# prime-slam/octreelib

Measured on AMD Instinct MI355X. Metric: Mpoints/s insert+subdivide+RANSAC, higher is better.
Workload: dtype f64; 1 GPU; BASELINE config 3: Grid 1 m voxels, 10000000 planar points per GPU (scene 32x32x32 voxels), insert + subdivide(len>64) + map_leaf_points_cuda_ransac(H=1024, k=6, thr=0.01, poses_per_batch=10) incl. apply_mask; points_per_gpu=10000000, K=64, hypotheses=1024, leaves=575543

## Files before the change

### octreelib_amd/csrc/common.h

```cpp
#pragma once

#include <hip/hip_runtime.h>
#include <stdint.h>

#include <cstdio>
#include <cstring>
#include <map>
#include <string>
#include <vector>

#include "../../include/octreelib_hip.h"

#include <atomic>
extern std::atomic<uint64_t> g_octl_host_syncs;
static inline hipError_t octl_counted_stream_sync(hipStream_t s) {
  g_octl_host_syncs.fetch_add(1, std::memory_order_relaxed);
  return hipStreamSynchronize(s);
}
static inline hipError_t octl_counted_event_sync(hipEvent_t e) {
  g_octl_host_syncs.fetch_add(1, std::memory_order_relaxed);
  return hipEventSynchronize(e);
}
#define hipStreamSynchronize(s) octl_counted_stream_sync(s)
#define hipEventSynchronize(e) octl_counted_event_sync(e)
// ... 81 lines not shown
  hipEvent_t self_gate = nullptr, self_done = nullptr;
  struct Upload { const char* dst; size_t bytes; hipEvent_t done; };
  std::vector<Upload> uploads;
  std::vector<DevBuf> pool;
  size_t pool_bytes = 0;
  std::map<void*, size_t> user_blocks;
  unsigned char geom_hint[192] = {0};
  bool geom_hint_valid = false;
  bool geom_hint_staged = false;
  struct octl_forest* pending_mask_forest = nullptr;
  uint64_t geom_hint_want = 0;
  bool geom_hint_two_pass = false;
  bool geom_sparse = false;
  bool had_chunks = false;
  int64_t spec_points = 0, spec_nodes = 0, spec_vox = 0, spec_blocks = 0;
  DevBuf hyp_dev;
  DevBuf f32_stage;
  DevBuf ls_buf;
  DevBuf rs_counters;
  int rs_parity = 0;
  uint32_t wait_seq = 0;
  bool rs_counters_dirty = false;
  std::vector<double> hyp_host;
  void* comm = nullptr;
  int n_ranks = 1, rank = 0;
  DevBuf routed_xyz, routed_gidx;
  bool routed_taken = false;
  DevBuf rt_hist, rt_counts, rt_matrix, rt_send_xyz, rt_send_gidx;
  int64_t routed_n = 0;
};

int octl_set_error(octl_ctx* ctx, int code, const char* fmt, ...);
enum { MIRROR_COPY_WORDS = 512, MIRROR_BBOX_WORD = 896, MIRROR_RS_VIOLATION = 990, MIRROR_MASK_TOTALS = 992,
       MIRROR_FLAG_BUILD = 1000, MIRROR_FLAG_MASK0 = 1001, MIRROR_FLAG_MASK1 = 1002 };
static_assert(MIRROR_COPY_WORDS <= MIRROR_BBOX_WORD && MIRROR_BBOX_WORD + 8 <= MIRROR_RS_VIOLATION &&
              MIRROR_RS_VIOLATION < MIRROR_MASK_TOTALS &&
              MIRROR_MASK_TOTALS + 2 <= MIRROR_FLAG_BUILD && MIRROR_FLAG_MASK1 < 1024, "mirror layout");
enum {
  SM_ERR = 0,
  SM_BBOX = 4,
  SM_NVOX = 12,
  SM_NSPLIT = 13,
  SM_NTILES = 14,
  SM_ETOTAL = 15,
  SM_NBLOCKS = 16,
  SM_BK_TICKET = 17,
// ... 95 lines not shown
```

### octreelib_amd/csrc/ctx.hip

```cpp
#include <chrono>
#include <cstdarg>
#include <cstdlib>

#include <algorithm>

#include "common.h"

int octl_set_error(octl_ctx* ctx, int code, const char* fmt, ...) {
  char buf[1024];
  va_list ap;
  va_start(ap, fmt);
  vsnprintf(buf, sizeof(buf), fmt, ap);
  va_end(ap);
  if (ctx) ctx->err = buf;
  return code;
}

std::atomic<uint64_t> g_octl_host_syncs{0};

namespace {
struct OptName { const char* name; int64_t OctlOptions::*field; };
const OptName kOptions[] = {
    {"NO_BUCKET_BUILD", &OctlOptions::no_bucket_build},     {"BUCKET_POINTS", &OctlOptions::bucket_points},
    {"SYNC_GEOM", &OctlOptions::sync_geom},                 {"NO_GEOM_HINT", &OctlOptions::no_geom_hint},
// ... 342 lines not shown
}

int octl_comm_destroy(octl_ctx* ctx);

void octl_ctx_destroy(octl_ctx* ctx) {
  if (!ctx) return;
  (void)hipSetDevice(ctx->device);
  (void)hipStreamSynchronize(ctx->stream);
  if (ctx->comm) (void)octl_comm_destroy(ctx);
  for (auto& pe : ctx->pending) {
    (void)hipEventDestroy(pe.start);
    (void)hipEventDestroy(pe.stop);
  }
  for (auto ev : ctx->event_pool) (void)hipEventDestroy(ev);
  if (ctx->handoff_event) (void)hipEventDestroy(ctx->handoff_event);
  for (auto ev : ctx->pin_event)
    if (ev) (void)hipEventDestroy(ev);
  for (auto& pb : ctx->pool) (void)hipFree(pb.p);
  ctx->pool.clear();
  for (auto& ub : ctx->user_blocks) (void)hipFree(ub.first);
  ctx->user_blocks.clear();
  for (auto& b : ctx->scan_tmp) devbuf_free(b);
  devbuf_free(ctx->hyp_dev);
  devbuf_free(ctx->f32_stage);
  devbuf_free(ctx->ls_buf);
  devbuf_free(ctx->rs_counters);
  devbuf_free(ctx->scan_status);
  devbuf_free(ctx->small);
  devbuf_free(ctx->routed_xyz);
  devbuf_free(ctx->routed_gidx);
  for (DevBuf* b : {&ctx->rt_hist, &ctx->rt_counts, &ctx->rt_matrix, &ctx->rt_send_xyz,
                    &ctx->rt_send_gidx})
    devbuf_free(*b);
  if (ctx->small_host) (void)hipHostFree(ctx->small_host);
  if (ctx->pinned) (void)hipHostFree(ctx->pinned);
  if (ctx->self_stream) {
    (void)hipStreamSynchronize(ctx->self_stream);
    (void)hipStreamDestroy(ctx->self_stream);
    if (ctx->self_gate) (void)hipEventDestroy(ctx->self_gate);
    if (ctx->self_done) (void)hipEventDestroy(ctx->self_done);
  }
  if (ctx->copy_stream) {
    (void)hipStreamSynchronize(ctx->copy_stream);
    (void)hipStreamDestroy(ctx->copy_stream);
  }
  if (ctx->copy_gate) (void)hipEventDestroy(ctx->copy_gate);
// ... 163 lines not shown
```

### octreelib_amd/csrc/forest.h

```cpp
#pragma once
#include "common.h"

#define OCTL_VOX_BIAS (1 << 20)
#define OCTL_VOX_ABS_LIMIT (1 << 30)
#define OCTL_VOX_DEAD (~0ull)
struct VoxOrg {
  int32_t x = 0, y = 0, z = 0;
};
__host__ __device__ static inline uint64_t vkey_pack(int64_t qx, int64_t qy, int64_t qz, const VoxOrg& g) {
  return ((uint64_t)(qx - g.x + OCTL_VOX_BIAS) << 42) | ((uint64_t)(qy - g.y + OCTL_VOX_BIAS) << 21) |
         (uint64_t)(qz - g.z + OCTL_VOX_BIAS);
}
__host__ __device__ static inline bool vkey_in_window(int64_t qx, int64_t qy, int64_t qz, const VoxOrg& g) {
  const int64_t ax = qx - g.x, ay = qy - g.y, az = qz - g.z;
  return ax > -OCTL_VOX_BIAS && ax < OCTL_VOX_BIAS && ay > -OCTL_VOX_BIAS && ay < OCTL_VOX_BIAS &&
         az > -OCTL_VOX_BIAS && az < OCTL_VOX_BIAS;
}
__host__ __device__ static inline void vkey_decode(uint64_t k, const VoxOrg& g, int64_t q[3]) {
  q[0] = (int64_t)((k >> 42) & 0x1FFFFF) - OCTL_VOX_BIAS + g.x;
  q[1] = (int64_t)((k >> 21) & 0x1FFFFF) - OCTL_VOX_BIAS + g.y;
  q[2] = (int64_t)(k & 0x1FFFFF) - OCTL_VOX_BIAS + g.z;
}

struct NodeTable {
// ... 82 lines not shown
  DevBuf bk_table;
  DevBuf bk_tot;
  DevBuf bk_chunks;
  DevBuf bk_vox;
  DevBuf bk_node;
  DevBuf leafinfo;
  struct LevelSeg { int64_t a, b; int depth; };
  std::vector<LevelSeg> level_segs;
  DevBuf vkey, path, lin[2], val[2], hist, idxbuf[2], pathbuf[2], flags, entries, split[2],
      split_tiles[2], child_sc, pose_off_dev, scheme_dev, root_up;
};

int forest_build(octl_forest* f, int64_t K, const uint8_t* scheme_mask, int32_t n_mask,
                 int32_t keep_scheme, int32_t max_depth, octl_build_info* info, const PlanarRule* planar = nullptr);
int planar_level_stats(octl_forest* f, const PlanarRule& rule, NodeTable& nt, int64_t first_new, int64_t n_new,
                       const uint32_t* idx, const double* xyz, int xs, int64_t n_alive);
int nodes_reserve(octl_ctx* ctx, NodeTable& t, int64_t cap);
void nodes_free(octl_ctx* ctx, NodeTable& t);

int ransac_launch(octl_ctx* ctx, const double* xyz_dev, int64_t n_points,
                  const uint32_t* blk_start, const int32_t* blk_size, const int32_t* order_dev,
                  int64_t nb, const double* hyp_dev, int32_t H, int32_t k, double thr,
                  uint8_t* mask_dev, float* plane_dev, int32_t* count_dev, int32_t* index_dev,
                  uint8_t* evaluated_dev, DevBuf& scratch, int64_t max_block = INT64_MAX);
int ransac_check_table(octl_ctx* ctx, const double* hyp, int32_t H, int32_t k);
int store_adopt(octl_forest* f, DevBuf& src, int64_t n, bool* adopted);
int store_compute_bbox(octl_forest* f);
int store_materialize(octl_forest* f);
int bbox_ensure(octl_forest* f);
int alive_ensure(octl_forest* f);
int forest_make_blocks(octl_forest* f);
int forest_finish_blocks(octl_forest* f, uint32_t* err_out);
int forest_sync_vkeys(octl_forest* f);
int forest_fix_origin(octl_forest* f, const int bb[6]);
int forest_sync_vcodes(octl_forest* f);
int forest_insert_incremental(octl_forest* f, int* done, octl_build_info* info);

int forest_settle(octl_forest* f);
void forest_forget_pending(octl_forest* f);
int ensure_mask(octl_forest* f);
```

### octreelib_amd/csrc/mask.hip

```cpp
#include "forest.h"
#include "lookback.h"

namespace {

__device__ __forceinline__ void mask_tile_count(const uint8_t* __restrict__ mask, int64_t n,
                                                uint32_t* __restrict__ tilecnt, uint32_t tile,
                                                uint8_t* __restrict__ alive_fill) {
  __shared__ uint32_t s_w[4];
  const int64_t i0 = (int64_t)tile * 2048 + (int64_t)threadIdx.x * 8;
  uint32_t c = 0;
  if (i0 + 8 <= n) {
    const uint64_t w = *reinterpret_cast<const uint64_t*>(mask + i0);
    const uint64_t nz = ((w & 0x7F7F7F7F7F7F7F7Full) + 0x7F7F7F7F7F7F7F7Full) | w;
    c = (uint32_t)__popcll(nz & 0x8080808080808080ull);
    if (alive_fill) *reinterpret_cast<uint64_t*>(alive_fill + i0) = 0x0101010101010101ull;
  } else {
    for (int64_t i = i0; i < n; ++i) {
      c += mask[i] ? 1u : 0u;
      if (alive_fill) alive_fill[i] = 1;
    }
  }
#pragma unroll
  for (int off = 32; off > 0; off >>= 1) c += __shfl_xor(c, off);
  if ((threadIdx.x & 63) == 0) s_w[threadIdx.x >> 6] = c;
// ... 94 lines not shown
    if ((keepbits >> r) & 1u) {
      const int64_t d = (int64_t)toff + s_cnt[r * 4 + wave] + rk[r];
      ord_idx2[d] = iv[r];
      xyz_ord2[3 * d] = px[r];
      xyz_ord2[3 * d + 1] = py[r];
      xyz_ord2[3 * d + 2] = pz[r];
      if (alive_fill) alive_fill[iv[r]] = 1;
    } else {
      alive[iv[r]] = 0;
    }
  }
}

__global__ __launch_bounds__(256) void k_compact_tiles(
    const uint8_t* __restrict__ mask, const uint32_t* __restrict__ tile_off, int64_t n,
    const uint32_t* __restrict__ ord_idx, const double* __restrict__ xyz_ord,
    uint32_t* __restrict__ ord_idx2, double* __restrict__ xyz_ord2, uint8_t* __restrict__ alive) {
  __shared__ uint32_t s_cnt[33];
  compact_tile(blockIdx.x, mask, n, ord_idx, xyz_ord, ord_idx2, xyz_ord2, alive, nullptr, s_cnt,
               [&](uint32_t) { return tile_off[blockIdx.x]; });
}


__global__ __launch_bounds__(256) void k_mask_scan(
    const uint8_t* __restrict__ mask, int64_t n, uint32_t nt,
    const uint32_t* __restrict__ ord_idx, const double* __restrict__ xyz_ord,
    uint32_t* __restrict__ ord_idx2, double* __restrict__ xyz_ord2, uint8_t* __restrict__ alive,
    const uint32_t* __restrict__ blk_start, const int32_t* __restrict__ blk_size, int64_t nb,
    const int32_t* __restrict__ blk_node, const int32_t* __restrict__ blk_slot, int32_t* __restrict__ blk_node2,
    int32_t* __restrict__ blk_slot2, uint32_t* __restrict__ blk_start2, int32_t* __restrict__ blk_size2,
    uint64_t* __restrict__ st_tiles, uint64_t* __restrict__ st_kept, uint64_t* __restrict__ st_ids, uint32_t epoch,
    uint32_t* __restrict__ mirror, uint32_t seq, uint8_t* __restrict__ alive_fill) {
  __shared__ uint32_t s_w[2][4];
  __shared__ uint32_t s_excl;
  __shared__ uint32_t s_cnt[33];
  const int lane = threadIdx.x & 63, wave = threadIdx.x >> 6;
  if (blockIdx.x < nt) {
    const uint32_t tile = blockIdx.x;
    compact_tile(tile, mask, n, ord_idx, xyz_ord, ord_idx2, xyz_ord2, alive, alive_fill, s_cnt,
                 [&](uint32_t total) {
                   const uint32_t excl = lookback_exclusive(st_tiles, epoch, tile, total, &s_excl);
                   if (threadIdx.x == 0 && tile == nt - 1) {
                     mirror[MIRROR_MASK_TOTALS] = excl + total;
                     mirror_publish(mirror, MIRROR_FLAG_MASK0, seq);
                   }
                   return excl;
                 });
    return;
  }
  const uint32_t bw = blockIdx.x - nt;
  const int64_t b = (int64_t)bw * 256 + threadIdx.x;
  const uint32_t st = b < nb ? blk_start[b] : 0u;
  const int sz = b < nb ? blk_size[b] : 0;
  uint32_t c = 0;
  if (sz <= 256)
    for (int i = 0; i < sz; ++i) c += mask[(size_t)st + i] ? 1u : 0u;
  unsigned long long big = __ballot(sz > 256);
  while (big) {
    const int src = __ffsll((long long)big) - 1;
    big &= big - 1;
    const uint32_t s0 = (uint32_t)__shfl((int)st, src);
    const int z = __shfl(sz, src);
    uint32_t cc = 0;
    for (int i = lane; i < z; i += 64) cc += mask[(size_t)s0 + i] ? 1u : 0u;
#pragma unroll
    for (int off = 32; off > 0; off >>= 1) cc += __shfl_xor(cc, off);
    if (lane == src) c = cc;
  }
  const uint32_t ne = c ? 1u : 0u;
  uint32_t ic = c, ie = ne;
#pragma unroll
  for (int off = 1; off < 64; off <<= 1) {
    const uint32_t tc = __shfl_up(ic, off), te = __shfl_up(ie, off);
    if (lane >= off) {
      ic += tc;
      ie += te;
    }
  }
  if (lane == 63) {
    s_w[0][wave] = ic;
    s_w[1][wave] = ie;
  }
  __syncthreads();
  uint32_t pc = ic - c, pe = ie - ne, tot_c = 0, tot_e = 0;
#pragma unroll
  for (int w = 0; w < 4; ++w) {
    if (w < wave) {
      pc += s_w[0][w];
      pe += s_w[1][w];
    }
    tot_c += s_w[0][w];
    tot_e += s_w[1][w];
  }
  __syncthreads();
  const uint32_t ex_c = lookback_exclusive(st_kept, epoch, bw, tot_c, &s_excl);
  __syncthreads();
  const uint32_t ex_e = lookback_exclusive(st_ids, epoch, bw, tot_e, &s_excl);
  if (threadIdx.x == 0 && bw == gridDim.x - nt - 1) {
    mirror[MIRROR_MASK_TOTALS + 1] = ex_e + tot_e;
    mirror_publish(mirror, MIRROR_FLAG_MASK1, seq);
  }
  if (b < nb && c) {
    const uint32_t id = ex_e + pe;
    blk_node2[id] = blk_node[b];
    blk_slot2[id] = blk_slot[b];
    blk_start2[id] = ex_c + pc;
    blk_size2[id] = (int32_t)c;
  }
}

__global__ __launch_bounds__(256) void k_blk_compact(
    const uint32_t* __restrict__ raw, const uint32_t* __restrict__ scanned, const uint32_t* __restrict__ grand_total,
    int64_t nt, int64_t nb, const int32_t* __restrict__ blk_node,
    const int32_t* __restrict__ blk_slot, int32_t* __restrict__ blk_node2, int32_t* __restrict__ blk_slot2,
    uint32_t* __restrict__ blk_start2, int32_t* __restrict__ blk_size2, uint32_t* __restrict__ mirror,
    uint32_t seq) {
  const int64_t b = (int64_t)blockIdx.x * blockDim.x + threadIdx.x;
  const uint32_t base_kept = scanned[nt], base_id = scanned[nt + nb];
  if (b == 0) {
    mirror[MIRROR_MASK_TOTALS] = base_id - base_kept;
    mirror[MIRROR_MASK_TOTALS + 1] = *grand_total - base_id;
    mirror_publish(mirror, MIRROR_FLAG_MASK0, seq);
    mirror_publish(mirror, MIRROR_FLAG_MASK1, seq);
  }
  if (b >= nb) return;
  const uint32_t c = raw[nt + b];
  if (!c) return;
  const uint32_t id = scanned[nt + nb + b] - base_id;
  blk_node2[id] = blk_node[b];
  blk_slot2[id] = blk_slot[b];
// ... 14 lines not shown
  for (int64_t i = threadIdx.x & 63; i < n; i += 64) mask[s0 + i] = 0;
}

int apply_device_mask(octl_forest* f, int64_t* n_alive_out, bool async = false) {
  octl_ctx* ctx = f->ctx;
  hipStream_t st = ctx->stream;
  if (ctx->pending_mask_forest && ctx->pending_mask_forest != f) OCTL_TRY(forest_settle(ctx->pending_mask_forest));
  OCTL_TRY(forest_settle(f));
  const int64_t n = f->n_ord, nb = f->n_blocks;
  f->mask_valid = false;
  f->fast_order_valid = false;
  f->pooled_valid = false;
  if (n > 0 && nb > 0) {
    KTimer t(ctx, "apply_mask");
    uint32_t* small = ctx->small.as<uint32_t>();
    const int64_t nt = ceil_div(n, 2048);
    const int64_t n_all = nt + 2 * nb;
    const size_t o_out = (((size_t)n_all + 8) * 4 + 15) & ~(size_t)15;
    OCTL_TRY(devbuf_reserve(ctx, f->flags, 2 * o_out));
    uint32_t* raw = f->flags.as<uint32_t>();
    uint32_t* scanned = reinterpret_cast<uint32_t*>(static_cast<char*>(f->flags.p) + o_out);
    const uint8_t* mask = f->mask.as<uint8_t>();
    const bool fused = !ctx->opt.no_fused_tables && nt + 2 * ceil_div(nb, 256) <= 1024;
    const uint32_t wait_seq = octl_wait_next_seq(ctx);
    uint8_t* fill = nullptr;
    if (f->alive_stale && f->n_ord == f->n_store) {
      fill = f->alive.as<uint8_t>();
      f->alive_stale = false;
    } else {
      OCTL_TRY(alive_ensure(f));
    }
    if (!fused) {
      OCTL_LAUNCH(k_blk_kept, dim3((unsigned)nt + grid_for(nb)), dim3(256), 0, st, mask, n, (uint32_t)nt, raw,
                         (const uint32_t*)f->blk_start.as<uint32_t>(), (const int32_t*)f->blk_size.as<int32_t>(), nb,
                         raw + nt, raw + nt + nb, fill);
      HIP_TRY(ctx, hipGetLastError());
      OCTL_TRY(octl_exclusive_scan_u32(ctx, raw, scanned, n_all, small + SM_MASK_TOTAL));
    }
    OCTL_TRY(devbuf_reserve(ctx, f->ord_idx2, (size_t)n * 4));
    OCTL_TRY(devbuf_reserve(ctx, f->xyz_ord2, (size_t)n * 24));
    OCTL_TRY(devbuf_reserve(ctx, f->blk_node2, (size_t)n * 4));
    OCTL_TRY(devbuf_reserve(ctx, f->blk_slot2, (size_t)n * 4));
    OCTL_TRY(devbuf_reserve(ctx, f->blk_start2, (size_t)n * 4));
    OCTL_TRY(devbuf_reserve(ctx, f->blk_size2, (size_t)n * 4));
    if (fused) {
      const int64_t nbw = ceil_div(nb, 256);
      uint64_t* status = nullptr;
      uint32_t epoch = 0;
      OCTL_TRY(octl_scan_status_acquire(ctx, nt + 2 * nbw, &status, &epoch));
      OCTL_LAUNCH(k_mask_scan, dim3((unsigned)(nt + nbw)), dim3(256), 0, st, mask, n, (uint32_t)nt,
                         (const uint32_t*)f->ord_idx.as<uint32_t>(), (const double*)f->xyz_ord.as<double>(),
                         f->ord_idx2.as<uint32_t>(), f->xyz_ord2.as<double>(), f->alive.as<uint8_t>(),
                         (const uint32_t*)f->blk_start.as<uint32_t>(), (const int32_t*)f->blk_size.as<int32_t>(), nb,
                         (const int32_t*)f->blk_node.as<int32_t>(), (const int32_t*)f->blk_slot.as<int32_t>(),
                         f->blk_node2.as<int32_t>(), f->blk_slot2.as<int32_t>(), f->blk_start2.as<uint32_t>(),
                         f->blk_size2.as<int32_t>(), status, status + nt, status + nt + nbw, epoch,
                         static_cast<uint32_t*>(ctx->small_host), wait_seq, fill);
      HIP_TRY(ctx, hipGetLastError());
    }
    if (!fused) {
      OCTL_LAUNCH(k_compact_tiles, dim3((unsigned)nt), dim3(256), 0, st, mask, (const uint32_t*)scanned, n,
                         (const uint32_t*)f->ord_idx.as<uint32_t>(), (const double*)f->xyz_ord.as<double>(),
                         f->ord_idx2.as<uint32_t>(), f->xyz_ord2.as<double>(), f->alive.as<uint8_t>());
      HIP_TRY(ctx, hipGetLastError());
      OCTL_LAUNCH(k_blk_compact, dim3(grid_for(nb)), dim3(256), 0, st, (const uint32_t*)raw,
                         (const uint32_t*)scanned, (const uint32_t*)(small + SM_MASK_TOTAL), nt, nb,
                         (const int32_t*)f->blk_node.as<int32_t>(), (const int32_t*)f->blk_slot.as<int32_t>(),
                         f->blk_node2.as<int32_t>(), f->blk_slot2.as<int32_t>(), f->blk_start2.as<uint32_t>(),
                         f->blk_size2.as<int32_t>(), static_cast<uint32_t*>(ctx->small_host), wait_seq);
      HIP_TRY(ctx, hipGetLastError());
    }
    std::swap(f->ord_idx, f->ord_idx2);
    std::swap(f->xyz_ord, f->xyz_ord2);
    std::swap(f->blk_node, f->blk_node2);
    std::swap(f->blk_slot, f->blk_slot2);
    std::swap(f->blk_start, f->blk_start2);
    std::swap(f->blk_size, f->blk_size2);
    f->totals_pending = true;
    f->totals_seq = wait_seq;
    f->totals_n_before = n;
    ctx->pending_mask_forest = f;
    if (!async) OCTL_TRY(forest_settle(f));
  }
  if (n_alive_out) *n_alive_out = f->n_ord;
  return OCTL_OK;
}

// ... 117 lines not shown
```

### octreelib_amd/csrc/order.hip

```cpp
#include <algorithm>

#include "forest.h"

namespace {

__global__ __launch_bounds__(256) void k_sub_up(const int32_t* __restrict__ first_child,
                                                int64_t a, int64_t b,
                                                uint32_t* __restrict__ nint) {
  const int64_t x = a + (int64_t)blockIdx.x * blockDim.x + threadIdx.x;
  if (x >= b) return;
  const int32_t fc = first_child[x];
  uint32_t s = 0;
  if (fc >= 0) {
    s = 1;
#pragma unroll
    for (int j = 0; j < 8; ++j) s += nint[fc + j];
  }
  nint[x] = s;
}

__global__ __launch_bounds__(256) void k_rank_down(const int32_t* __restrict__ first_child,
                                                   int64_t a, int64_t b,
                                                   const uint32_t* __restrict__ nint,
                                                   uint32_t* __restrict__ rank) {
// ... 283 lines not shown

extern "C" int octl_forest_ransac_all(octl_forest* f, int32_t poses_per_batch, const int32_t* e0,
                                      int32_t n_e0, const double* hypotheses, int32_t H, int32_t k,
                                      double threshold) {
  if (!f || !hypotheses) return OCTL_E_INVALID;
  OCTL_TRY(forest_settle(f));
  bool mask_fresh = false;
  const int rc = ransac_all_impl(f, poses_per_batch, e0, n_e0, hypotheses, H, k, threshold, &mask_fresh);
  if (mask_fresh) f->mask_valid = (rc == OCTL_OK);
  return rc;
}

static int ransac_all_impl(octl_forest* f, int32_t poses_per_batch, const int32_t* e0, int32_t n_e0,
                           const double* hypotheses, int32_t H, int32_t k, double threshold,
                           bool* mask_fresh) {
  octl_ctx* ctx = f->ctx;
  if (!f->built) return octl_set_error(ctx, OCTL_E_STATE, "ransac before build");
  if (poses_per_batch < 1) return octl_set_error(ctx, OCTL_E_INVALID, "poses_per_batch < 1");
  if (H < 1 || H > 1024 || k < 1) return octl_set_error(ctx, OCTL_E_INVALID, "bad H or k");
  OCTL_TRY(ransac_check_table(ctx, hypotheses, H, k));
  const int n_poses = (int)f->pose_off.size() - 1;
  if (e0 && n_e0 != n_poses) return octl_set_error(ctx, OCTL_E_INVALID, "e0 size mismatch");
  HIP_TRY(ctx, hipSetDevice(ctx->device));
  hipStream_t st = ctx->stream;
  if (!f->mask_valid) {
    OCTL_TRY(devbuf_reserve(ctx, f->mask, (size_t)std::max<int64_t>(f->n_ord, 1)));
    *mask_fresh = true;
  }
  if (f->n_blocks == 0) return OCTL_OK;
  const size_t hyp_cap_before = ctx->hyp_dev.cap;
  OCTL_TRY(devbuf_reserve(ctx, ctx->hyp_dev, (size_t)H * k * 8));
  const bool same_table = hyp_cap_before == ctx->hyp_dev.cap && ctx->hyp_host.size() == (size_t)H * k &&
                          std::memcmp(ctx->hyp_host.data(), hypotheses, (size_t)H * k * 8) == 0;
  if (same_table) {
  } else if ((size_t)H * k * 8 <= 64 * 1024) {
    char* pin = static_cast<char*>(ctx->pinned) + 128 * 1024;
    OCTL_TRY(pin_region_wait(ctx, 1));
    std::memcpy(pin, hypotheses, (size_t)H * k * 8);
    OCTL_TRY(octl_copy_from_pinned(ctx, ctx->hyp_dev.p, pin, (size_t)H * k * 8));
    OCTL_TRY(pin_region_mark(ctx, 1));
  } else {
    HIP_TRY(ctx, hipMemcpyAsync(ctx->hyp_dev.p, hypotheses, (size_t)H * k * 8, hipMemcpyHostToDevice, st));
    HIP_TRY(ctx, hipStreamSynchronize(st));
  }
  if (!same_table) ctx->hyp_host.assign(hypotheses, hypotheses + (size_t)H * k);
  const bool one_batch = n_poses <= poses_per_batch;
  std::vector<uint32_t> slot_counts;
  OCTL_TRY(forest_reference_order(f, e0, slot_counts, !one_batch));
  if (one_batch) {
    OCTL_TRY(ransac_launch(ctx, f->xyz_ord.as<double>(), f->n_ord, f->blk_start.as<uint32_t>(),
                           f->blk_size.as<int32_t>(), f->rs_order.as<int32_t>(), f->n_blocks,
                           ctx->hyp_dev.as<double>(), H, k, threshold, f->mask.as<uint8_t>(), nullptr,
                           nullptr, nullptr, nullptr, f->rs_scratch, f->max_block_hint));
    return OCTL_OK;
  }
  int64_t off = 0;
  for (int p0 = 0; p0 < n_poses; p0 += poses_per_batch) {
    int64_t nbatch = 0;
    for (int p = p0; p < std::min(n_poses, p0 + poses_per_batch); ++p) nbatch += slot_counts[p];
    if (nbatch > 0)
      OCTL_TRY(ransac_launch(ctx, f->xyz_ord.as<double>(), f->n_ord, f->blk_start.as<uint32_t>(),
                             f->blk_size.as<int32_t>(), f->rs_order.as<int32_t>() + off, nbatch,
                             ctx->hyp_dev.as<double>(), H, k, threshold, f->mask.as<uint8_t>(),
                             nullptr, nullptr, nullptr, nullptr, f->rs_scratch, f->max_block_hint));
    off += nbatch;
  }
  return OCTL_OK;
}
```

### octreelib_amd/csrc/ransac.hip

```cpp
#include <algorithm>
#include <cstdlib>
#include <type_traits>

#include "forest.h"
#include "lookback.h"
#include "wave_utils.h"

namespace {

__device__ __forceinline__ double div_by_small_int(double c, int k) {
  const double kd = (double)k;
  const double zh = 1.0 / kd;
  const double zl = fma(-kd, zh, 1.0) / kd;
  const double a = fabs(c);
  if (!((int(a > 1e-290) | int(c == 0.0)) & int(a < 1e290))) return c / kd;
  return copysign(fma(c, zh, c * zl), c);
}

__device__ __forceinline__ bool coord_in_fast_range(double v) {
  const uint32_t hi = (uint32_t)__double2hiint(v), lo = (uint32_t)__double2loint(v);
  const uint32_t e = (hi >> 20) & 0x7FFu;
  return (e - (1023u - 30u)) <= 60u || (hi | lo) == 0u;
}

// ... 1317 lines not shown
  if (bins[threadIdx.x]) atomicAdd(&counters[RC_BINS + threadIdx.x], bins[threadIdx.x]);
}

__device__ __forceinline__ void pos_table_entry(const double* __restrict__ hyp, int H, int k,
                                                uint2* __restrict__ tab, int n, int t) {
  const double* __restrict__ row = hyp + (int64_t)t * k;
  uint32_t x = 0, y = 0;
  for (int i = 0; i < k; ++i) {
    bool risky;
    const uint32_t g = (uint32_t)sample_index_cached(row[i], n, &risky);
    if (i < 4) x |= g << (8 * i); else y |= g << (8 * (i - 4));
    y |= (risky || g == (uint32_t)n) ? (0x10000u << i) : 0u;
  }
  tab[(size_t)n * (size_t)H + t] = uint2{x, y};
}
__device__ __forceinline__ void pos_table_part(const double* __restrict__ hyp, int H, int k,
                                               const uint32_t* __restrict__ counters, uint2* __restrict__ tab,
                                               int n, int part) {
  const int t = part * 256 + (int)threadIdx.x;
  if (t >= H || n < k || counters[RC_BINS + n] == 0u) return;
  pos_table_entry(hyp, H, k, tab, n, t);
}

__global__ __launch_bounds__(256) void k_block_scatter(const BlockDesc* __restrict__ desc, int64_t nb,
                                                       int cap, int k,
                                                       uint32_t* __restrict__ counters,
                                                       BlockDesc* __restrict__ sdesc, unsigned n_scatter,
                                                       const double* __restrict__ hyp, int H,
                                                       uint2* __restrict__ tab, uint32_t* __restrict__ next_counters) {
  if (next_counters && blockIdx.x == gridDim.x - 1)
    for (int w = threadIdx.x; w < RC_WORDS; w += blockDim.x) next_counters[w] = 0;
  if (blockIdx.x >= n_scatter) {
    const unsigned parts = (unsigned)(H + 255) / 256u;
    const unsigned id = blockIdx.x - n_scatter;
    pos_table_part(hyp, H, k, counters, tab, (int)(id / parts), (int)(id % parts));
    return;
  }
  __shared__ uint32_t cnt[256];
  __shared__ uint32_t base[256];
  __shared__ uint32_t c[256];
  cnt[threadIdx.x] = 0;
  c[threadIdx.x] = counters[RC_BINS + threadIdx.x];
  __syncthreads();
  uint32_t first = 0;
  for (int m = 255; m > (int)threadIdx.x; --m) first += c[m];
  if (blockIdx.x == 0) {
// ... 139 lines not shown
    first[m] = f;
    counters[RC_BINS + m] = cm;
    counters[RC_START + m] = f;
    if (m == 0) counters[RC_SORTED] = f + cm;
  }
  __syncthreads();
#pragma unroll
  for (int r = 0; r < BPS_PER_THREAD; ++r)
    if (dd[r].n >= 0) sdesc[first[dd[r].n] + rank[r]] = dd[r];
}

}

int ransac_check_table(octl_ctx* ctx, const double* hyp, int32_t H, int32_t k) {
  const int64_t n = (int64_t)H * k;
  for (int64_t i = 0; i < n; ++i)
    if (!(hyp[i] >= 0.0 && hyp[i] < 1.0))
      return octl_set_error(ctx, OCTL_E_INVALID,
                            "hypothesis table entry %lld = %g is outside [0, 1): the table must hold "
                            "np.random.random draws (cuda_ransac.py:39-41)", (long long)i, hyp[i]);
  return OCTL_OK;
}

int ransac_launch(octl_ctx* ctx, const double* xyz_dev, int64_t n_points,
                  const uint32_t* blk_start, const int32_t* blk_size, const int32_t* order_dev,
                  int64_t nb, const double* hyp_dev, int32_t H, int32_t k, double thr,
                  uint8_t* mask_dev, float* plane_dev, int32_t* count_dev, int32_t* index_dev,
                  uint8_t* evaluated_dev, DevBuf& scratch, int64_t max_block) {
  (void)evaluated_dev;
  if (nb <= 0) return OCTL_OK;
  if (H < 1 || H > 1024) return octl_set_error(ctx, OCTL_E_INVALID, "H must be in [1, 1024]");
  if (k < 1) return octl_set_error(ctx, OCTL_E_INVALID, "initial_points_number must be positive");
  const bool any_k = k > RS_KMAX;
  if (nb >= ((int64_t)1 << 31)) return octl_set_error(ctx, OCTL_E_INVALID, "too many blocks");
  hipStream_t st = ctx->stream;
  const size_t off_d = (((size_t)nb + 8) * 4 + 31) & ~(size_t)31;
  const size_t off_s = off_d + (size_t)nb * sizeof(BlockDesc);
  const size_t off_b = off_s + (size_t)nb * sizeof(BlockDesc);
  const size_t off_c = (off_b + (size_t)nb * 4 + 31) & ~(size_t)31;
  const bool use_tab = !any_k && k >= 3 && k <= 6 && (H > 256 || k == 6);
  const size_t off_t = (off_c + RC_WORDS * 4 + 31) & ~(size_t)31;
  OCTL_TRY(devbuf_reserve(ctx, scratch, off_t + (use_tab ? (size_t)256 * (size_t)H * sizeof(uint2) : 0)));
  char* base = static_cast<char*>(scratch.p);
  uint32_t* tmp = scratch.as<uint32_t>();
  BlockDesc* desc = reinterpret_cast<BlockDesc*>(base + off_d);
  BlockDesc* sdesc = reinterpret_cast<BlockDesc*>(base + off_s);
  uint32_t* big_list = reinterpret_cast<uint32_t*>(base + off_b);
  uint32_t* counters = reinterpret_cast<uint32_t*>(base + off_c);
  const bool fused = !ctx->opt.no_fused_tables;
  uint32_t* next_counters = nullptr;
  if (fused) {
    if (!ctx->rs_counters.p || ctx->rs_counters_dirty) {
      OCTL_TRY(devbuf_reserve(ctx, ctx->rs_counters, (size_t)2 * RC_WORDS * 4));
      HIP_TRY(ctx, hipMemsetAsync(ctx->rs_counters.p, 0, (size_t)2 * RC_WORDS * 4, st));
      ctx->rs_parity = 0;
    }
    counters = ctx->rs_counters.as<uint32_t>() + (size_t)ctx->rs_parity * RC_WORDS;
    next_counters = ctx->rs_counters.as<uint32_t>() + (size_t)(ctx->rs_parity ^ 1) * RC_WORDS;
    ctx->rs_parity ^= 1;
    ctx->rs_counters_dirty = true;
  }
  uint2* pos_tab = use_tab ? reinterpret_cast<uint2*>(base + off_t) : nullptr;
  const int threads = (H <= 64) ? 64 : (H <= 256 ? 256 : RS_BIG_THREADS);
  RansacOut out{mask_dev, plane_dev, count_dev, index_dev};
  if (fused && nb <= BPS_MAX) {
    KTimer t(ctx, "ransac_prepare");
    const int cap = any_k ? 0 : threads - 1;
    const unsigned n_table = use_tab && cap >= k ? (unsigned)(cap - k + 1) * (unsigned)ceil_div(H, BPS_THREADS) : 0u;
    auto kp = nb <= 2 * BPS_THREADS ? k_block_prepare_small<2>
              : (nb <= 4 * BPS_THREADS ? k_block_prepare_small<4>
                                       : (nb <= 6 * BPS_THREADS ? k_block_prepare_small<6> : k_block_prepare_small<8>));
    OCTL_LAUNCH(kp, dim3(1 + n_table), dim3(BPS_THREADS), 0, st, order_dev, blk_start, blk_size, nb,
                       n_points, cap, (int)k, desc, sdesc, big_list, counters, out, max_block,
                       static_cast<uint32_t*>(ctx->small_host), hyp_dev, (int)H, pos_tab, next_counters);
    HIP_TRY(ctx, hipGetLastError());
    ctx->rs_counters_dirty = false;
  } else {
    KTimer t(ctx, "ransac_prepare");
    if (fused) {
      const unsigned g = (unsigned)ceil_div(nb, 256 * BP_PER_THREAD);
      uint64_t* status = nullptr;
      uint32_t epoch = 0;
      OCTL_TRY(octl_scan_status_acquire(ctx, g, &status, &epoch));
      OCTL_LAUNCH(k_block_prepare, dim3(g), dim3(256), 0, st, order_dev, blk_start, blk_size, nb, n_points,
                         any_k ? 0 : threads - 1, (int)k, desc, big_list, counters, out, status, epoch, max_block,
                         static_cast<uint32_t*>(ctx->small_host));
      HIP_TRY(ctx, hipGetLastError());
    } else {
      const unsigned g = (unsigned)ceil_div(nb, 256);
      OCTL_LAUNCH(k_block_sizes_in_order, dim3(g), dim3(256), 0, st, order_dev, blk_size, nb, tmp, counters);
      HIP_TRY(ctx, hipGetLastError());
      OCTL_TRY(octl_exclusive_scan_u32(ctx, tmp, tmp, nb, nullptr));
      OCTL_LAUNCH(k_block_desc, dim3((unsigned)ceil_div(nb, 256 * BD_PER_THREAD)), dim3(256), 0, st, order_dev,
                         blk_start, blk_size,
                         (const uint32_t*)tmp, nb, n_points, any_k ? 0 : threads - 1, (int)k, desc, big_list,
                         counters, out);
      HIP_TRY(ctx, hipGetLastError());
    }
    const unsigned n_scatter = (unsigned)ceil_div(nb, 256 * BS_PER_THREAD);
    const unsigned n_table = use_tab ? 256u * (unsigned)ceil_div(H, 256) : 0u;
    OCTL_LAUNCH(k_block_scatter, dim3(n_scatter + n_table), dim3(256), 0, st,
                       (const BlockDesc*)desc, nb, any_k ? 0 : threads - 1, (int)k, counters, sdesc, n_scatter, hyp_dev,
                       (int)H, pos_tab, next_counters);
    HIP_TRY(ctx, hipGetLastError());
    ctx->rs_counters_dirty = false;
  }
  const int cus = octl_ctx_cus(ctx);
  KTimer t(ctx, "ransac");
  hipStream_t side = st;
  bool on_side = false;
  int waves_per_block = (int)ctx->opt.ransac_waves;
  if (waves_per_block == 0 && !any_k && H > 256) {
    const int64_t slots = (int64_t)cus * 16;
    if (nb * 2 <= slots) waves_per_block = 4;
    else if (nb <= 6 * slots) waves_per_block = 2;
  }
  const bool need_small = max_block >= RS_TINY_THREADS, need_mid = max_block >= RS_SMALL_THREADS,
             need_big = any_k || max_block >= threads;
  const bool side_work = waves_per_block == 4 ? need_big
                         : (waves_per_block == 2 ? (need_mid || need_big) : (need_small || need_mid || need_big));
  if (!any_k && H > 256 && side_work && octl_ctx_side_stream(ctx) &&
      hipEventRecord(ctx->self_gate, st) == hipSuccess &&
      hipStreamWaitEvent(ctx->self_stream, ctx->self_gate, 0) == hipSuccess) {
    side = ctx->self_stream;
    on_side = true;
  }
  const int no_prescreen = ctx->opt.no_ransac_prescreen ? 1 : 0;
#define OCTL_RANSAC_RANGE(THREADS, HPL, KT, PER_CU, LO, HI, PT, ST)                              \
  do {                                                                                           \
    const unsigned g = (unsigned)std::min<int64_t>(nb, (int64_t)cus * (PER_CU));                 \
    if (H == (THREADS) * (HPL))                                                                  \
      OCTL_LAUNCH((k_ransac<THREADS, HPL, KT, true, PT>), dim3(g), dim3(THREADS), 0, ST,         \
                         xyz_dev, (const BlockDesc*)sdesc, (const uint32_t*)(LO), (const uint32_t*)(HI), \
                         hyp_dev, H, k, thr, out, (const uint2*)pos_tab, no_prescreen);           \
    else                                                                                         \
      OCTL_LAUNCH((k_ransac<THREADS, HPL, KT, false, PT>), dim3(g), dim3(THREADS), 0, ST,        \
                         xyz_dev, (const BlockDesc*)sdesc, (const uint32_t*)(LO), (const uint32_t*)(HI), \
                         hyp_dev, H, k, thr, out, (const uint2*)pos_tab, no_prescreen);           \
  } while (0)
#define OCTL_RANSAC_LAUNCH(THREADS, HPL, KT, PER_CU, PT) \
  OCTL_RANSAC_RANGE(THREADS, HPL, KT, PER_CU, nullptr, counters + RC_SORTED, PT, st)
#define OCTL_RANSAC_SPLIT(KT)                                                                                    \
  do {                                                                                                           \
    if (waves_per_block == 4) {                                                                                  \
      OCTL_RANSAC_RANGE(RS_BIG_THREADS, RS_BIG_HPL, KT, RS_PER_CU, nullptr, counters + RC_SORTED, true, st);     \
    } else if (waves_per_block == 2) {                                                                           \
      if (need_mid)                                                                                              \
        OCTL_RANSAC_RANGE(RS_BIG_THREADS, RS_BIG_HPL, KT, RS_PER_CU, nullptr,                                    \
                          counters + RC_START + RS_SMALL_THREADS - 1, true, side);                               \
      HIP_TRY(ctx, hipGetLastError());                                                                           \
      OCTL_RANSAC_RANGE(RS_SMALL_THREADS, (1024 / RS_SMALL_THREADS), KT, RS_SMALL_PER_CU,                        \
                        counters + RC_START + RS_SMALL_THREADS - 1, counters + RC_SORTED, true, st);             \
    } else {                                                                                                     \
      if (need_mid)                                                                                              \
        OCTL_RANSAC_RANGE(RS_BIG_THREADS, RS_BIG_HPL, KT, RS_PER_CU, nullptr,                                    \
                          counters + RC_START + RS_SMALL_THREADS - 1, true, side);                               \
      HIP_TRY(ctx, hipGetLastError());                                                                           \
      if (need_small)                                                                                            \
        OCTL_RANSAC_RANGE(RS_SMALL_THREADS, (1024 / RS_SMALL_THREADS), KT, RS_SMALL_PER_CU,                      \
                          counters + RC_START + RS_SMALL_THREADS - 1, counters + RC_START + RS_TINY_THREADS - 1, \
                          true, side);                                                                           \
// ... 136 lines not shown
```

Measured before the change: 3556 Mpoints/s.

## Cache RANSAC position table across calls and add tiled mask-head scan kernel

Result: no change. 3546 Mpoints/s (-0.3%).

```diff
diff --git a/octreelib_amd/csrc/common.h b/octreelib_amd/csrc/common.h
--- a/octreelib_amd/csrc/common.h
+++ b/octreelib_amd/csrc/common.h
@@ -127,6 +127,10 @@
   uint32_t wait_seq = 0;
   bool rs_counters_dirty = false;
   std::vector<double> hyp_host;
+  int32_t hyp_H = 0, hyp_k = 0;
+  uint64_t hyp_hash = 0;
+  DevBuf pos_tab;
+  bool pos_tab_valid = false;
   void* comm = nullptr;
   int n_ranks = 1, rank = 0;
   DevBuf routed_xyz, routed_gidx;
diff --git a/octreelib_amd/csrc/ctx.hip b/octreelib_amd/csrc/ctx.hip
--- a/octreelib_amd/csrc/ctx.hip
+++ b/octreelib_amd/csrc/ctx.hip
@@ -388,6 +388,7 @@
   ctx->user_blocks.clear();
   for (auto& b : ctx->scan_tmp) devbuf_free(b);
   devbuf_free(ctx->hyp_dev);
+  devbuf_free(ctx->pos_tab);
   devbuf_free(ctx->f32_stage);
   devbuf_free(ctx->ls_buf);
   devbuf_free(ctx->rs_counters);
diff --git a/octreelib_amd/csrc/forest.h b/octreelib_amd/csrc/forest.h
--- a/octreelib_amd/csrc/forest.h
+++ b/octreelib_amd/csrc/forest.h
@@ -128,7 +128,11 @@
                   const uint32_t* blk_start, const int32_t* blk_size, const int32_t* order_dev,
                   int64_t nb, const double* hyp_dev, int32_t H, int32_t k, double thr,
                   uint8_t* mask_dev, float* plane_dev, int32_t* count_dev, int32_t* index_dev,
-                  uint8_t* evaluated_dev, DevBuf& scratch, int64_t max_block = INT64_MAX);
+                  uint8_t* evaluated_dev, DevBuf& scratch, int64_t max_block = INT64_MAX,
+                  const uint2* pos_tab_cached = nullptr);
+uint64_t ransac_table_hash(const double* hyp, int64_t n_values);
+bool ransac_table_cached(const octl_ctx* ctx, const double* hyp, int32_t H, int32_t k, uint64_t hash);
+int ransac_table_acquire(octl_ctx* ctx, const double* hyp, int32_t H, int32_t k, const uint2** pos_tab);
 int ransac_check_table(octl_ctx* ctx, const double* hyp, int32_t H, int32_t k);
 int store_adopt(octl_forest* f, DevBuf& src, int64_t n, bool* adopted);
 int store_compute_bbox(octl_forest* f);
diff --git a/octreelib_amd/csrc/mask.hip b/octreelib_amd/csrc/mask.hip
--- a/octreelib_amd/csrc/mask.hip
+++ b/octreelib_amd/csrc/mask.hip
@@ -140,33 +140,14 @@
 }
 
 
-__global__ __launch_bounds__(256) void k_mask_scan(
-    const uint8_t* __restrict__ mask, int64_t n, uint32_t nt,
-    const uint32_t* __restrict__ ord_idx, const double* __restrict__ xyz_ord,
-    uint32_t* __restrict__ ord_idx2, double* __restrict__ xyz_ord2, uint8_t* __restrict__ alive,
+__device__ __forceinline__ void compact_block_table(
+    uint32_t bw, uint32_t n_bw, const uint8_t* __restrict__ mask,
     const uint32_t* __restrict__ blk_start, const int32_t* __restrict__ blk_size, int64_t nb,
     const int32_t* __restrict__ blk_node, const int32_t* __restrict__ blk_slot, int32_t* __restrict__ blk_node2,
     int32_t* __restrict__ blk_slot2, uint32_t* __restrict__ blk_start2, int32_t* __restrict__ blk_size2,
-    uint64_t* __restrict__ st_tiles, uint64_t* __restrict__ st_kept, uint64_t* __restrict__ st_ids, uint32_t epoch,
-    uint32_t* __restrict__ mirror, uint32_t seq, uint8_t* __restrict__ alive_fill) {
-  __shared__ uint32_t s_w[2][4];
-  __shared__ uint32_t s_excl;
-  __shared__ uint32_t s_cnt[33];
+    uint64_t* __restrict__ st_kept, uint64_t* __restrict__ st_ids, uint32_t epoch, uint32_t* __restrict__ mirror,
+    uint32_t seq, uint32_t (*s_w)[4], uint32_t* s_excl) {
   const int lane = threadIdx.x & 63, wave = threadIdx.x >> 6;
-  if (blockIdx.x < nt) {
-    const uint32_t tile = blockIdx.x;
-    compact_tile(tile, mask, n, ord_idx, xyz_ord, ord_idx2, xyz_ord2, alive, alive_fill, s_cnt,
-                 [&](uint32_t total) {
-                   const uint32_t excl = lookback_exclusive(st_tiles, epoch, tile, total, &s_excl);
-                   if (threadIdx.x == 0 && tile == nt - 1) {
-                     mirror[MIRROR_MASK_TOTALS] = excl + total;
-                     mirror_publish(mirror, MIRROR_FLAG_MASK0, seq);
-                   }
-                   return excl;
-                 });
-    return;
-  }
-  const uint32_t bw = blockIdx.x - nt;
   const int64_t b = (int64_t)bw * 256 + threadIdx.x;
   const uint32_t st = b < nb ? blk_start[b] : 0u;
   const int sz = b < nb ? blk_size[b] : 0;
@@ -211,10 +192,10 @@
     tot_e += s_w[1][w];
   }
   __syncthreads();
-  const uint32_t ex_c = lookback_exclusive(st_kept, epoch, bw, tot_c, &s_excl);
-  __syncthreads();
-  const uint32_t ex_e = lookback_exclusive(st_ids, epoch, bw, tot_e, &s_excl);
-  if (threadIdx.x == 0 && bw == gridDim.x - nt - 1) {
+  const uint32_t ex_c = lookback_exclusive(st_kept, epoch, bw, tot_c, s_excl);
+  __syncthreads();
+  const uint32_t ex_e = lookback_exclusive(st_ids, epoch, bw, tot_e, s_excl);
+  if (threadIdx.x == 0 && bw == n_bw - 1) {
     mirror[MIRROR_MASK_TOTALS + 1] = ex_e + tot_e;
     mirror_publish(mirror, MIRROR_FLAG_MASK1, seq);
   }
@@ -224,6 +205,91 @@
     blk_slot2[id] = blk_slot[b];
     blk_start2[id] = ex_c + pc;
     blk_size2[id] = (int32_t)c;
+  }
+}
+
+__global__ __launch_bounds__(256) void k_mask_scan(
+    const uint8_t* __restrict__ mask, int64_t n, uint32_t nt,
+    const uint32_t* __restrict__ ord_idx, const double* __restrict__ xyz_ord,
+    uint32_t* __restrict__ ord_idx2, double* __restrict__ xyz_ord2, uint8_t* __restrict__ alive,
+    const uint32_t* __restrict__ blk_start, const int32_t* __restrict__ blk_size, int64_t nb,
+    const int32_t* __restrict__ blk_node, const int32_t* __restrict__ blk_slot, int32_t* __restrict__ blk_node2,
+    int32_t* __restrict__ blk_slot2, uint32_t* __restrict__ blk_start2, int32_t* __restrict__ blk_size2,
+    uint64_t* __restrict__ st_tiles, uint64_t* __restrict__ st_kept, uint64_t* __restrict__ st_ids, uint32_t epoch,
+    uint32_t* __restrict__ mirror, uint32_t seq, uint8_t* __restrict__ alive_fill) {
+  __shared__ uint32_t s_w[2][4];
+  __shared__ uint32_t s_excl;
+  __shared__ uint32_t s_cnt[33];
+  if (blockIdx.x < nt) {
+    const uint32_t tile = blockIdx.x;
+    compact_tile(tile, mask, n, ord_idx, xyz_ord, ord_idx2, xyz_ord2, alive, alive_fill, s_cnt,
+                 [&](uint32_t total) {
+                   const uint32_t excl = lookback_exclusive(st_tiles, epoch, tile, total, &s_excl);
+                   if (threadIdx.x == 0 && tile == nt - 1) {
+                     mirror[MIRROR_MASK_TOTALS] = excl + total;
+                     mirror_publish(mirror, MIRROR_FLAG_MASK0, seq);
+                   }
+                   return excl;
+                 });
+    return;
+  }
+  compact_block_table(blockIdx.x - nt, gridDim.x - nt, mask, blk_start, blk_size, nb, blk_node, blk_slot, blk_node2,
+                      blk_slot2, blk_start2, blk_size2, st_kept, st_ids, epoch, mirror, seq, s_w, &s_excl);
+}
+
+constexpr int MH_TILES = 8;
+__global__ __launch_bounds__(256) void k_mask_head(
+    const uint8_t* __restrict__ mask, int64_t n, uint32_t nt, uint32_t ntg, uint32_t* __restrict__ tile_off,
+    const uint32_t* __restrict__ blk_start, const int32_t* __restrict__ blk_size, int64_t nb,
+    const int32_t* __restrict__ blk_node, const int32_t* __restrict__ blk_slot, int32_t* __restrict__ blk_node2,
+    int32_t* __restrict__ blk_slot2, uint32_t* __restrict__ blk_start2, int32_t* __restrict__ blk_size2,
+    uint64_t* __restrict__ st_tiles, uint64_t* __restrict__ st_kept, uint64_t* __restrict__ st_ids, uint32_t epoch,
+    uint32_t* __restrict__ mirror, uint32_t seq, uint8_t* __restrict__ alive_fill) {
+  __shared__ uint32_t s_w[2][4];
+  __shared__ uint32_t s_excl;
+  __shared__ uint32_t s_t[MH_TILES][4];
+  if (blockIdx.x >= ntg) {
+    compact_block_table(blockIdx.x - ntg, gridDim.x - ntg, mask, blk_start, blk_size, nb, blk_node, blk_slot,
+                        blk_node2, blk_slot2, blk_start2, blk_size2, st_kept, st_ids, epoch, mirror, seq, s_w, &s_excl);
+    return;
+  }
+  const int lane = threadIdx.x & 63, wave = threadIdx.x >> 6;
+  const uint32_t tile0 = blockIdx.x * MH_TILES;
+  uint32_t c[MH_TILES];
+#pragma unroll
+  for (int r = 0; r < MH_TILES; ++r) {
+    const int64_t i0 = (int64_t)(tile0 + r) * 2048 + (int64_t)threadIdx.x * 8;
+    c[r] = 0;
+    if (i0 + 8 <= n) {
+      const uint64_t w = *reinterpret_cast<const uint64_t*>(mask + i0);
+      const uint64_t nz = ((w & 0x7F7F7F7F7F7F7F7Full) + 0x7F7F7F7F7F7F7F7Full) | w;
+      c[r] = (uint32_t)__popcll(nz & 0x8080808080808080ull);
+      if (alive_fill) *reinterpret_cast<uint64_t*>(alive_fill + i0) = 0x0101010101010101ull;
+    } else {
+      for (int64_t i = i0; i < n; ++i) {
+        c[r] += mask[i] ? 1u : 0u;
+        if (alive_fill) alive_fill[i] = 1;
+      }
+    }
+  }
+#pragma unroll
+  for (int r = 0; r < MH_TILES; ++r) {
+#pragma unroll
+    for (int off = 32; off > 0; off >>= 1) c[r] += __shfl_xor(c[r], off);
+    if (lane == 0) s_t[r][wave] = c[r];
+  }
+  __syncthreads();
+  uint32_t before = 0, total = 0;
+#pragma unroll
+  for (int r = 0; r < MH_TILES; ++r) {
+    if (r == (int)threadIdx.x) before = total;
+    total += s_t[r][0] + s_t[r][1] + s_t[r][2] + s_t[r][3];
+  }
+  const uint32_t excl = lookback_exclusive(st_tiles, epoch, blockIdx.x, total, &s_excl);
+  if (threadIdx.x < MH_TILES && tile0 + threadIdx.x < nt) tile_off[tile0 + threadIdx.x] = excl + before;
+  if (threadIdx.x == 0 && blockIdx.x == ntg - 1) {
+    mirror[MIRROR_MASK_TOTALS] = excl + total;
+    mirror_publish(mirror, MIRROR_FLAG_MASK0, seq);
   }
 }
 
@@ -284,6 +350,7 @@
     uint32_t* scanned = reinterpret_cast<uint32_t*>(static_cast<char*>(f->flags.p) + o_out);
     const uint8_t* mask = f->mask.as<uint8_t>();
     const bool fused = !ctx->opt.no_fused_tables && nt + 2 * ceil_div(nb, 256) <= 1024;
+    const bool head = !ctx->opt.no_fused_tables && !fused;
     const uint32_t wait_seq = octl_wait_next_seq(ctx);
     uint8_t* fill = nullptr;
     if (f->alive_stale && f->n_ord == f->n_store) {
@@ -292,7 +359,7 @@
     } else {
       OCTL_TRY(alive_ensure(f));
     }
-    if (!fused) {
+    if (!fused && !head) {
       OCTL_LAUNCH(k_blk_kept, dim3((unsigned)nt + grid_for(nb)), dim3(256), 0, st, mask, n, (uint32_t)nt, raw,
                          (const uint32_t*)f->blk_start.as<uint32_t>(), (const int32_t*)f->blk_size.as<int32_t>(), nb,
                          raw + nt, raw + nt + nb, fill);
@@ -320,11 +387,27 @@
                          static_cast<uint32_t*>(ctx->small_host), wait_seq, fill);
       HIP_TRY(ctx, hipGetLastError());
     }
+    if (head) {
+      const int64_t ntg = ceil_div(nt, MH_TILES), nbw = ceil_div(nb, 256);
+      uint64_t* status = nullptr;
+      uint32_t epoch = 0;
+      OCTL_TRY(octl_scan_status_acquire(ctx, ntg + 2 * nbw, &status, &epoch));
+      OCTL_LAUNCH(k_mask_head, dim3((unsigned)(ntg + nbw)), dim3(256), 0, st, mask, n, (uint32_t)nt, (uint32_t)ntg,
+                         scanned, (const uint32_t*)f->blk_start.as<uint32_t>(),
+                         (const int32_t*)f->blk_size.as<int32_t>(), nb, (const int32_t*)f->blk_node.as<int32_t>(),
+                         (const int32_t*)f->blk_slot.as<int32_t>(), f->blk_node2.as<int32_t>(),
+                         f->blk_slot2.as<int32_t>(), f->blk_start2.as<uint32_t>(), f->blk_size2.as<int32_t>(), status,
+                         status + ntg, status + ntg + nbw, epoch, static_cast<uint32_t*>(ctx->small_host), wait_seq,
+                         fill);
+      HIP_TRY(ctx, hipGetLastError());
+    }
     if (!fused) {
       OCTL_LAUNCH(k_compact_tiles, dim3((unsigned)nt), dim3(256), 0, st, mask, (const uint32_t*)scanned, n,
                          (const uint32_t*)f->ord_idx.as<uint32_t>(), (const double*)f->xyz_ord.as<double>(),
                          f->ord_idx2.as<uint32_t>(), f->xyz_ord2.as<double>(), f->alive.as<uint8_t>());
       HIP_TRY(ctx, hipGetLastError());
+    }
+    if (!fused && !head) {
       OCTL_LAUNCH(k_blk_compact, dim3(grid_for(nb)), dim3(256), 0, st, (const uint32_t*)raw,
                          (const uint32_t*)scanned, (const uint32_t*)(small + SM_MASK_TOTAL), nt, nb,
                          (const int32_t*)f->blk_node.as<int32_t>(), (const int32_t*)f->blk_slot.as<int32_t>(),
diff --git a/octreelib_amd/csrc/order.hip b/octreelib_amd/csrc/order.hip
--- a/octreelib_amd/csrc/order.hip
+++ b/octreelib_amd/csrc/order.hip
@@ -329,28 +329,13 @@
   const int n_poses = (int)f->pose_off.size() - 1;
   if (e0 && n_e0 != n_poses) return octl_set_error(ctx, OCTL_E_INVALID, "e0 size mismatch");
   HIP_TRY(ctx, hipSetDevice(ctx->device));
-  hipStream_t st = ctx->stream;
   if (!f->mask_valid) {
     OCTL_TRY(devbuf_reserve(ctx, f->mask, (size_t)std::max<int64_t>(f->n_ord, 1)));
     *mask_fresh = true;
   }
   if (f->n_blocks == 0) return OCTL_OK;
-  const size_t hyp_cap_before = ctx->hyp_dev.cap;
-  OCTL_TRY(devbuf_reserve(ctx, ctx->hyp_dev, (size_t)H * k * 8));
-  const bool same_table = hyp_cap_before == ctx->hyp_dev.cap && ctx->hyp_host.size() == (size_t)H * k &&
-                          std::memcmp(ctx->hyp_host.data(), hypotheses, (size_t)H * k * 8) == 0;
-  if (same_table) {
-  } else if ((size_t)H * k * 8 <= 64 * 1024) {
-    char* pin = static_cast<char*>(ctx->pinned) + 128 * 1024;
-    OCTL_TRY(pin_region_wait(ctx, 1));
-    std::memcpy(pin, hypotheses, (size_t)H * k * 8);
-    OCTL_TRY(octl_copy_from_pinned(ctx, ctx->hyp_dev.p, pin, (size_t)H * k * 8));
-    OCTL_TRY(pin_region_mark(ctx, 1));
-  } else {
-    HIP_TRY(ctx, hipMemcpyAsync(ctx->hyp_dev.p, hypotheses, (size_t)H * k * 8, hipMemcpyHostToDevice, st));
-    HIP_TRY(ctx, hipStreamSynchronize(st));
-  }
-  if (!same_table) ctx->hyp_host.assign(hypotheses, hypotheses + (size_t)H * k);
+  const uint2* pos_tab = nullptr;
+  OCTL_TRY(ransac_table_acquire(ctx, hypotheses, H, k, &pos_tab));
   const bool one_batch = n_poses <= poses_per_batch;
   std::vector<uint32_t> slot_counts;
   OCTL_TRY(forest_reference_order(f, e0, slot_counts, !one_batch));
@@ -358,7 +343,7 @@
     OCTL_TRY(ransac_launch(ctx, f->xyz_ord.as<double>(), f->n_ord, f->blk_start.as<uint32_t>(),
                            f->blk_size.as<int32_t>(), f->rs_order.as<int32_t>(), f->n_blocks,
                            ctx->hyp_dev.as<double>(), H, k, threshold, f->mask.as<uint8_t>(), nullptr,
-                           nullptr, nullptr, nullptr, f->rs_scratch, f->max_block_hint));
+                           nullptr, nullptr, nullptr, f->rs_scratch, f->max_block_hint, pos_tab));
     return OCTL_OK;
   }
   int64_t off = 0;
@@ -369,7 +354,7 @@
       OCTL_TRY(ransac_launch(ctx, f->xyz_ord.as<double>(), f->n_ord, f->blk_start.as<uint32_t>(),
                              f->blk_size.as<int32_t>(), f->rs_order.as<int32_t>() + off, nbatch,
                              ctx->hyp_dev.as<double>(), H, k, threshold, f->mask.as<uint8_t>(),
-                             nullptr, nullptr, nullptr, nullptr, f->rs_scratch, f->max_block_hint));
+                             nullptr, nullptr, nullptr, nullptr, f->rs_scratch, f->max_block_hint, pos_tab));
     off += nbatch;
   }
   return OCTL_OK;
diff --git a/octreelib_amd/csrc/ransac.hip b/octreelib_amd/csrc/ransac.hip
--- a/octreelib_amd/csrc/ransac.hip
+++ b/octreelib_amd/csrc/ransac.hip
@@ -1,5 +1,6 @@
 #include <algorithm>
 #include <cstdlib>
+#include <cstring>
 #include <type_traits>
 
 #include "forest.h"
@@ -1363,6 +1364,13 @@
   pos_table_entry(hyp, H, k, tab, n, t);
 }
 
+__global__ __launch_bounds__(256) void k_pos_table_build(const double* __restrict__ hyp, int H, int k,
+                                                         uint2* __restrict__ tab) {
+  const int parts = (H + 255) / 256;
+  const int n = k + (int)blockIdx.x / parts, t = ((int)blockIdx.x % parts) * 256 + (int)threadIdx.x;
+  if (t < H && n <= 255) pos_table_entry(hyp, H, k, tab, n, t);
+}
+
 __global__ __launch_bounds__(256) void k_block_scatter(const BlockDesc* __restrict__ desc, int64_t nb,
                                                        int cap, int k,
                                                        uint32_t* __restrict__ counters,
@@ -1548,11 +1556,72 @@
   return OCTL_OK;
 }
 
+static bool ransac_uses_pos_table(int32_t H, int32_t k) {
+  return k >= 3 && k <= 6 && (H > 256 || k == 6);
+}
+
+uint64_t ransac_table_hash(const double* hyp, int64_t n_values) {
+  uint64_t h[4] = {0x9E3779B97F4A7C15ull, 0xC2B2AE3D27D4EB4Full, 0x165667B19E3779F9ull, 0x27D4EB2F165667C5ull};
+  for (int64_t i = 0; i < n_values; ++i) {
+    uint64_t w;
+    std::memcpy(&w, hyp + i, 8);
+    uint64_t& l = h[i & 3];
+    l = (l ^ w) * 0x100000001B3ull;
+    l ^= l >> 29;
+  }
+  uint64_t r = (uint64_t)n_values;
+  for (int j = 0; j < 4; ++j) r = (r ^ h[j]) * 0xFF51AFD7ED558CCDull, r ^= r >> 32;
+  return r;
+}
+
+bool ransac_table_cached(const octl_ctx* ctx, const double* hyp, int32_t H, int32_t k, uint64_t hash) {
+  const size_t n = (size_t)H * (size_t)k;
+  return ctx->hyp_dev.p && ctx->hyp_H == H && ctx->hyp_k == k && ctx->hyp_hash == hash &&
+         ctx->hyp_host.size() == n && std::memcmp(ctx->hyp_host.data(), hyp, n * 8) == 0;
+}
+
+int ransac_table_acquire(octl_ctx* ctx, const double* hyp, int32_t H, int32_t k, const uint2** pos_tab) {
+  hipStream_t st = ctx->stream;
+  const size_t bytes = (size_t)H * k * 8;
+  const uint64_t hash = ransac_table_hash(hyp, (int64_t)H * k);
+  if (!ransac_table_cached(ctx, hyp, H, k, hash)) {
+    ctx->hyp_host.clear();
+    ctx->pos_tab_valid = false;
+    OCTL_TRY(devbuf_reserve(ctx, ctx->hyp_dev, bytes));
+    if (bytes <= 64 * 1024) {
+      char* pin = static_cast<char*>(ctx->pinned) + 128 * 1024;
+      OCTL_TRY(pin_region_wait(ctx, 1));
+      std::memcpy(pin, hyp, bytes);
+      OCTL_TRY(octl_copy_from_pinned(ctx, ctx->hyp_dev.p, pin, bytes));
+      OCTL_TRY(pin_region_mark(ctx, 1));
+    } else {
+      HIP_TRY(ctx, hipMemcpyAsync(ctx->hyp_dev.p, hyp, bytes, hipMemcpyHostToDevice, st));
+      HIP_TRY(ctx, hipStreamSynchronize(st));
+    }
+    ctx->hyp_host.assign(hyp, hyp + (size_t)H * k);
+    ctx->hyp_H = H;
+    ctx->hyp_k = k;
+    ctx->hyp_hash = hash;
+  }
+  *pos_tab = nullptr;
+  if (!ransac_uses_pos_table(H, k)) return OCTL_OK;
+  if (!ctx->pos_tab_valid) {
+    OCTL_TRY(devbuf_reserve(ctx, ctx->pos_tab, (size_t)256 * (size_t)H * sizeof(uint2)));
+    const unsigned parts = (unsigned)ceil_div(H, 256);
+    OCTL_LAUNCH(k_pos_table_build, dim3((unsigned)(255 - k + 1) * parts), dim3(256), 0, st,
+                       (const double*)ctx->hyp_dev.as<double>(), (int)H, (int)k, ctx->pos_tab.as<uint2>());
+    HIP_TRY(ctx, hipGetLastError());
+    ctx->pos_tab_valid = true;
+  }
+  *pos_tab = ctx->pos_tab.as<uint2>();
+  return OCTL_OK;
+}
+
 int ransac_launch(octl_ctx* ctx, const double* xyz_dev, int64_t n_points,
                   const uint32_t* blk_start, const int32_t* blk_size, const int32_t* order_dev,
                   int64_t nb, const double* hyp_dev, int32_t H, int32_t k, double thr,
                   uint8_t* mask_dev, float* plane_dev, int32_t* count_dev, int32_t* index_dev,
-                  uint8_t* evaluated_dev, DevBuf& scratch, int64_t max_block) {
+                  uint8_t* evaluated_dev, DevBuf& scratch, int64_t max_block, const uint2* pos_tab_cached) {
   (void)evaluated_dev;
   if (nb <= 0) return OCTL_OK;
   if (H < 1 || H > 1024) return octl_set_error(ctx, OCTL_E_INVALID, "H must be in [1, 1024]");
@@ -1564,9 +1633,10 @@
   const size_t off_s = off_d + (size_t)nb * sizeof(BlockDesc);
   const size_t off_b = off_s + (size_t)nb * sizeof(BlockDesc);
   const size_t off_c = (off_b + (size_t)nb * 4 + 31) & ~(size_t)31;
-  const bool use_tab = !any_k && k >= 3 && k <= 6 && (H > 256 || k == 6);
+  const bool use_tab = ransac_uses_pos_table(H, k);
+  const bool make_tab = use_tab && !pos_tab_cached;
   const size_t off_t = (off_c + RC_WORDS * 4 + 31) & ~(size_t)31;
-  OCTL_TRY(devbuf_reserve(ctx, scratch, off_t + (use_tab ? (size_t)256 * (size_t)H * sizeof(uint2) : 0)));
+  OCTL_TRY(devbuf_reserve(ctx, scratch, off_t + (make_tab ? (size_t)256 * (size_t)H * sizeof(uint2) : 0)));
   char* base = static_cast<char*>(scratch.p);
   uint32_t* tmp = scratch.as<uint32_t>();
   BlockDesc* desc = reinterpret_cast<BlockDesc*>(base + off_d);
@@ -1586,19 +1656,20 @@
     ctx->rs_parity ^= 1;
     ctx->rs_counters_dirty = true;
   }
-  uint2* pos_tab = use_tab ? reinterpret_cast<uint2*>(base + off_t) : nullptr;
+  uint2* pos_tab_own = make_tab ? reinterpret_cast<uint2*>(base + off_t) : nullptr;
+  const uint2* pos_tab = make_tab ? pos_tab_own : (use_tab ? pos_tab_cached : nullptr);
   const int threads = (H <= 64) ? 64 : (H <= 256 ? 256 : RS_BIG_THREADS);
   RansacOut out{mask_dev, plane_dev, count_dev, index_dev};
   if (fused && nb <= BPS_MAX) {
     KTimer t(ctx, "ransac_prepare");
     const int cap = any_k ? 0 : threads - 1;
-    const unsigned n_table = use_tab && cap >= k ? (unsigned)(cap - k + 1) * (unsigned)ceil_div(H, BPS_THREADS) : 0u;
+    const unsigned n_table = make_tab && cap >= k ? (unsigned)(cap - k + 1) * (unsigned)ceil_div(H, BPS_THREADS) : 0u;
     auto kp = nb <= 2 * BPS_THREADS ? k_block_prepare_small<2>
               : (nb <= 4 * BPS_THREADS ? k_block_prepare_small<4>
                                        : (nb <= 6 * BPS_THREADS ? k_block_prepare_small<6> : k_block_prepare_small<8>));
     OCTL_LAUNCH(kp, dim3(1 + n_table), dim3(BPS_THREADS), 0, st, order_dev, blk_start, blk_size, nb,
                        n_points, cap, (int)k, desc, sdesc, big_list, counters, out, max_block,
-                       static_cast<uint32_t*>(ctx->small_host), hyp_dev, (int)H, pos_tab, next_counters);
+                       static_cast<uint32_t*>(ctx->small_host), hyp_dev, (int)H, pos_tab_own, next_counters);
     HIP_TRY(ctx, hipGetLastError());
     ctx->rs_counters_dirty = false;
   } else {
@@ -1624,10 +1695,10 @@
       HIP_TRY(ctx, hipGetLastError());
     }
     const unsigned n_scatter = (unsigned)ceil_div(nb, 256 * BS_PER_THREAD);
-    const unsigned n_table = use_tab ? 256u * (unsigned)ceil_div(H, 256) : 0u;
+    const unsigned n_table = make_tab ? 256u * (unsigned)ceil_div(H, 256) : 0u;
     OCTL_LAUNCH(k_block_scatter, dim3(n_scatter + n_table), dim3(256), 0, st,
                        (const BlockDesc*)desc, nb, any_k ? 0 : threads - 1, (int)k, counters, sdesc, n_scatter, hyp_dev,
-                       (int)H, pos_tab, next_counters);
+                       (int)H, pos_tab_own, next_counters);
     HIP_TRY(ctx, hipGetLastError());
     ctx->rs_counters_dirty = false;
   }
@@ -1658,11 +1729,11 @@
     if (H == (THREADS) * (HPL))                                                                  \
       OCTL_LAUNCH((k_ransac<THREADS, HPL, KT, true, PT>), dim3(g), dim3(THREADS), 0, ST,         \
                          xyz_dev, (const BlockDesc*)sdesc, (const uint32_t*)(LO), (const uint32_t*)(HI), \
-                         hyp_dev, H, k, thr, out, (const uint2*)pos_tab, no_prescreen);           \
+                         hyp_dev, H, k, thr, out, pos_tab, no_prescreen);           \
     else                                                                                         \
       OCTL_LAUNCH((k_ransac<THREADS, HPL, KT, false, PT>), dim3(g), dim3(THREADS), 0, ST,        \
                          xyz_dev, (const BlockDesc*)sdesc, (const uint32_t*)(LO), (const uint32_t*)(HI), \
-                         hyp_dev, H, k, thr, out, (const uint2*)pos_tab, no_prescreen);           \
+                         hyp_dev, H, k, thr, out, pos_tab, no_prescreen);           \
   } while (0)
 #define OCTL_RANSAC_LAUNCH(THREADS, HPL, KT, PER_CU, PT) \
   OCTL_RANSAC_RANGE(THREADS, HPL, KT, PER_CU, nullptr, counters + RC_SORTED, PT, st)
```
